# haberdashPI/SignalOperators.jl

Hardware: NVIDIA B200
Metric: sink Msamples/s (Filt+resample+Mix chain) at 1/2/4/8 B200; % of HBM peak (higher is better)
Workload: dtype f64

## Files before the change

### signaloperators.jl_b200/csrc/k_fir_tmap.cuh

```cuda
#pragma once
#include <cuda.h>

#include <type_traits>

#include "k_fir_mma.cuh"

namespace sigops {

constexpr int kFtRows = 128;
constexpr int kFtSlotPos = 16;
constexpr int kFtSlotBytes = kFtRows * 128;
constexpr int kFtMaxSlots = 10;
constexpr int kFtNCW = 8, kFtNAW = 4;
constexpr int kFtThreads = 16 * 32;
constexpr int kFtRegsCompute = 176, kFtRegsHelper = 112, kFtRegsMisc = 40;
constexpr int kFtMaxKs = 64;

struct FirTmParams {
    double* scalars;
    int nscalars, sumsq_slot, nch;
    int64_t nrows, n_out;
    int tapsper;
    int ks;
    int nslot;
    int64_t ntiles, tiles_per_seg;
    const double* pfb;
    const double* dpfb;
    const int64_t* xi0;
    const int32_t* poff;
    const double* alpha;
    int tab_doubles;
    double gain;
    const double* bands_g;
    int period_tiles;
    int64_t epoch_tiles;
    int n_epochs;
    long long* dbg;
    int exp;
};

inline size_t fir_tm_smem_bytes(int nslot, int ks, int tab_doubles, bool has_dpfb) {
    return (size_t)nslot * kFtSlotBytes + 2 * 16384 + (size_t)2 * 4 * ks * 8 * sizeof(double) +
           (size_t)tab_doubles * sizeof(double) * (has_dpfb ? 2 : 1) + 1024;
}

__device__ __forceinline__ void tmap_load_2d(unsigned smem_dst, const CUtensorMap* tm, int c0, int c1, uint64_t* bar) {
    asm volatile("cp.async.bulk.tensor.2d.shared::cluster.global.mbarrier::complete_tx::bytes [%0], [%1, {%2, %3}], [%4];" ::"r"(smem_dst),
                 "l"(tm), "r"(c0), "r"(c1), "r"(smem_u32(bar))
                 : "memory");
}
__device__ __forceinline__ void tmap_store_2d(const CUtensorMap* tm, int c0, int c1, unsigned smem_src) {
    asm volatile("cp.async.bulk.tensor.2d.global.shared::cta.bulk_group [%0, {%1, %2}], [%3];" ::"l"(tm), "r"(c0), "r"(c1), "r"(smem_src)
                 : "memory");
}
__device__ __forceinline__ double lds_f64(unsigned a) {
    double v;
    asm volatile("ld.shared.f64 %0, [%1];" : "=d"(v) : "r"(a));
    return v;
}
__device__ __forceinline__ void sts_f64(unsigned a, double v) { asm volatile("st.shared.f64 [%0], %1;" ::"r"(a), "d"(v) : "memory"); }
__device__ __forceinline__ void sts_v2f64(unsigned a, double x, double y) {
    asm volatile("st.shared.v2.f64 [%0], {%1, %2};" ::"r"(a), "d"(x), "d"(y) : "memory");
}

__device__ __forceinline__ void mbar_wait_a(unsigned bar, unsigned parity) {
    asm volatile(
        "{\n"
        ".reg .pred p;\n"
        "LAB_WAIT:\n"
        "mbarrier.try_wait.parity.shared::cta.b64 p, [%0], %1;\n"
        "@p bra LAB_DONE;\n"
        "bra LAB_WAIT;\n"
        "LAB_DONE:\n"
        "}\n" ::"r"(bar), "r"(parity) : "memory");
}
__device__ __forceinline__ void mbar_arrive_a(unsigned bar) {
    asm volatile("mbarrier.arrive.shared::cta.b64 _, [%0];" ::"r"(bar) : "memory");
}

template <bool SSQ, bool DBG = false>
__global__ void __launch_bounds__(kFtThreads, 1)
k_fir_tmap(const __grid_constant__ FirTmParams P, const __grid_constant__ CUtensorMap tm_in,
           const __grid_constant__ CUtensorMap tm_out) {
    extern __shared__ unsigned char ft_smem_raw[];
    __shared__ uint64_t bar_full[kFtMaxSlots], bar_done[4], bar_taps[2], bar_stg_full[2], bar_stg_free[2];
    __shared__ unsigned done_count;

    const unsigned ring = (smem_u32(ft_smem_raw) + 1023u) & ~1023u;
    const unsigned stg = ring + (unsigned)P.nslot * kFtSlotBytes;
    const unsigned bands = stg + 2 * 16384;
    const unsigned tabs = bands + 2u * 4u * (unsigned)P.ks * 64u;

    const int tid = threadIdx.x, warp = tid >> 5, lane = tid & 31;
    const int row0 = (int)blockIdx.y * kFtRows;
    const int64_t t0 = (int64_t)blockIdx.x * P.tiles_per_seg;
    const int64_t t1 = (t0 + P.tiles_per_seg < P.ntiles) ? t0 + P.tiles_per_seg : P.ntiles;
    if (t0 >= t1) return;

    for (int i = tid; i < P.tab_doubles; i += kFtThreads) {
        sts_f64(tabs + 8u * i, __ldg(P.pfb + i) * P.gain);
        if (P.dpfb) sts_f64(tabs + 8u * (P.tab_doubles + i), __ldg(P.dpfb + i) * P.gain);
    }
    if (tid == 0) {
        done_count = 0u;
        for (int i = 0; i < P.nslot; ++i) mbar_init(&bar_full[i], 1);
        for (int i = 0; i < 4; ++i) mbar_init(&bar_done[i], kFtNCW);
        mbar_init(&bar_taps[0], P.bands_g ? 2 : kFtNAW * 32);
        mbar_init(&bar_taps[1], P.bands_g ? 2 : kFtNAW * 32);
        for (int i = 0; i < 2; ++i) {
            mbar_init(&bar_stg_full[i], kFtNCW / 2);
            mbar_init(&bar_stg_free[i], 1);
        }
        asm volatile("fence.mbarrier_init.release.cluster;" ::: "memory");
    }
    fence_async_smem();
    __syncthreads();

    const int64_t pos_base = (__ldg(P.xi0 + t0 * kFmT) - P.tapsper + 1) & ~int64_t(kFtSlotPos - 1);
    const unsigned band_tile = 4u * (unsigned)P.ks * 64u;

    if (warp < kFtNCW) {
        constexpr int F = 8;
        const int gw = warp & 3, rw = warp >> 2;
        asm volatile("setmaxnreg.inc.sync.aligned.u32 %0;" ::"n"(kFtRegsCompute));
        const int kk = lane & 3, rr = lane >> 2;
        const int rmap = ((rr & 1) << 2) | (rr & 2) | (rr >> 2);
        const int rloc = rw * (8 * F) + rmap;
        const int nn = rr ^ ((kk >> 1) << 2);
        unsigned key = (unsigned)rmap << 4;
        unsigned srow = stg + rloc * 128;
        unsigned bcol = (unsigned)((gw * P.ks + kk) * 64 + nn * 8);
        unsigned arow1 = ring + rloc * 128;
        unsigned ring_end = arow1 + (unsigned)P.nslot * kFtSlotBytes;
        unsigned a_taps = smem_u32(&bar_taps[0]), a_free = smem_u32(&bar_stg_free[rw]), a_full = smem_u32(&bar_stg_full[rw]);
        unsigned a_done = smem_u32(&bar_done[0]), a_cnt = smem_u32(&done_count), lead = lane == 0 ? 1u : 0u;
        asm volatile("" : "+r"(key), "+r"(srow), "+r"(bcol), "+r"(arow1), "+r"(ring_end));
        asm volatile("" : "+r"(a_taps), "+r"(a_free), "+r"(a_full), "+r"(a_done), "+r"(a_cnt), "+r"(lead));
        const int nt = (int)(t1 - t0);
        const int64_t* xp = P.xi0 + t0 * kFmT + 8 * gw;
        double ssq[SSQ ? 8 : 1];
#pragma unroll
        for (int i = 0; i < (SSQ ? 8 : 1); ++i) ssq[i] = 0.0;

        int64_t xq_nx, x7_nx;
        auto fetch_idx = [&](int u) {
            xq_nx = __ldg(xp + (int64_t)u * kFmT);
            x7_nx = __ldg(xp + (int64_t)u * kFmT + 7);
        };
        fetch_idx(0);
        long long dbg_acc[5] = {0, 0, 0, 0, 0};

        unsigned cur = arow1, nxt = arow1;
        int jcur = 0;
        unsigned off[4];
        bool w[4];
        unsigned bq = 0;
        int nbt = 0;
        struct Ops { double a[F], b; };
        Ops o0, o1;

        auto load_ops = [&](Ops& o, auto J) {
            const unsigned ap = (w[J.value] ? nxt : cur) + off[J.value];
#pragma unroll
            for (int i = 0; i < F; ++i) o.a[i] = lds_f64(ap + i * 1024);
            o.b = lds_f64(bq);
            bq += 256;
        };
        auto next_slot = [&]() {
            ++jcur;
            cur = nxt;
            nxt += kFtSlotBytes;
            if (nxt == ring_end) nxt = arow1;
        };
        auto setup = [&](int u, Ops& o) {
            const long long cs = DBG ? clock64() : 0;
            const int s = u & 1;
            const int r = (int)(xq_nx - P.tapsper + 1 - pos_base) + kk;
            int n = (int)(x7_nx - xq_nx) + P.tapsper + 3;
            n >>= 2;
            nbt = n < (P.ks >> 2) ? n : (P.ks >> 2);
            if (u + 1 < nt) fetch_idx(u + 1);
            const int j_new = r >> 4;
            int slot = (int)((cur - arow1) / kFtSlotBytes) + (j_new - jcur);
            while (slot >= P.nslot) slot -= P.nslot;
            while (slot < 0) slot += P.nslot;
            jcur = j_new;
            cur = arow1 + (unsigned)slot * kFtSlotBytes;
            nxt = cur + kFtSlotBytes;
            if (nxt == ring_end) nxt = arow1;
            const unsigned sub0 = (unsigned)(r & 15) << 3;
#pragma unroll
            for (int J = 0; J < 4; ++J) {
                const unsigned q = sub0 + 32u * J;
                w[J] = q >= 128u;
                off[J] = (q & 127u) ^ key;
            }
            bq = bands + s * band_tile + bcol;
            const long long c0 = DBG ? clock64() : 0;
            if (!(P.exp & 16)) mbar_wait_a(a_taps + 8u * s, (unsigned)(u >> 1) & 1u);
            if (DBG) dbg_acc[0] += clock64() - c0;
            load_ops(o, std::integral_constant<int, 0>{});
            if (DBG) dbg_acc[1] += clock64() - cs;
        };
        auto mma_block = [&](double (&acc)[F][2], const Ops& o) {
#pragma unroll
            for (int i = 0; i < F; ++i) dmma884(acc[i][0], acc[i][1], o.a[i], o.b);
        };
        auto stage_store = [&](double (&o)[F][2], int u_old) {
            const long long c0 = DBG ? clock64() : 0;
            if (u_old > 0) mbar_wait_a(a_free, (unsigned)(u_old - 1) & 1u);
            if (DBG) dbg_acc[2] += clock64() - c0;
            if (!(P.exp & 1)) {
                const unsigned sp = srow + (gw >> 1) * 16384 + ((unsigned)(((gw & 1) * 4 + kk) << 4) ^ key);
#pragma unroll
                for (int i = 0; i < F; ++i) sts_v2f64(sp + i * 1024, o[i][0], o[i][1]);
            }
            if (SSQ) {
#pragma unroll
                for (int i = 0; i < F; ++i) ssq[i] = fma(o[i][0], o[i][0], fma(o[i][1], o[i][1], ssq[i]));
            }
            if (DBG) dbg_acc[3] += clock64() - c0;
        };
        auto stage_signal = [&]() {
            const long long c0 = DBG ? clock64() : 0;
            fence_async_smem();
            __syncwarp();
            if (lead) mbar_arrive_a(a_full);
            if (DBG) dbg_acc[3] += clock64() - c0;
        };
        auto tile = [&](double (&acc)[F][2], double (&old)[F][2], int u) {
            const bool more = u + 1 < nt;
#pragma unroll
            for (int i = 0; i < F; ++i) acc[i][0] = acc[i][1] = 0.0;
            const int n = nbt;
            using I0 = std::integral_constant<int, 0>;
            using I1 = std::integral_constant<int, 1>;
            using I2 = std::integral_constant<int, 2>;
            using I3 = std::integral_constant<int, 3>;
            int b = 0;
            bool signalled = u == 0;
            while (true) {
                if (b + 1 < n) {
                    load_ops(o1, I1{});
                    mma_block(acc, o0);
                    if (b == 0 && u > 0) stage_store(old, u - 1);
                } else {
                    if (more) setup(u + 1, o1);
                    mma_block(acc, o0);
                    if (b == 0 && u > 0) stage_store(old, u - 1);
                    o0 = o1;
                    break;
                }
                ++b;
                if (b + 1 < n) {
                    load_ops(o0, I2{});
                    mma_block(acc, o1);
                } else {
                    if (more) setup(u + 1, o0);
                    mma_block(acc, o1);
                    break;
                }
                ++b;
                if (b + 1 < n) {
                    load_ops(o1, I3{});
                    mma_block(acc, o0);
                    if (b == 2 && u > 0) { stage_signal(); signalled = true; }
                } else {
                    if (more) setup(u + 1, o1);
                    mma_block(acc, o0);
                    o0 = o1;
                    break;
                }
                ++b;
                if (b + 1 < n) {
                    next_slot();
                    load_ops(o0, I0{});
                    mma_block(acc, o1);
                } else {
                    if (more) setup(u + 1, o0);
                    mma_block(acc, o1);
                    break;
                }
                ++b;
            }
            if (!signalled) stage_signal();
            __syncwarp();
            if (lead) {
                mbar_arrive_a(a_done + 8u * (u & 3));
                asm volatile("red.release.cta.shared::cta.add.u32 [%0], 1;" ::"r"(a_cnt) : "memory");
            }
        };

        double accA[F][2], accB[F][2];
        setup(0, o0);
        const long long cstart = DBG ? clock64() : 0;
        for (int u = 0; u < nt; u += 2) {
            tile(accA, accB, u);
            if (u + 1 < nt) tile(accB, accA, u + 1);
        }
        if (DBG && warp == 0 && lane == 0) {
            long long* d = P.dbg + ((size_t)blockIdx.y * gridDim.x + blockIdx.x) * 8;
            d[0] = dbg_acc[0]; d[1] = dbg_acc[1]; d[2] = dbg_acc[2]; d[3] = clock64() - cstart; d[6] = dbg_acc[3];
        }
        if (nt & 1) stage_store(accA, nt - 1);
        else stage_store(accB, nt - 1);
        stage_signal();
        if (SSQ) {
#pragma unroll
            for (int i = 0; i < F; ++i) {
                double v = ssq[i];
                v += __shfl_xor_sync(0xffffffffu, v, 1);
                v += __shfl_xor_sync(0xffffffffu, v, 2);
                const int64_t row = (int64_t)row0 + rloc + 8 * i;
                if (kk == 0 && row < P.nrows) atomicAdd(P.scalars + (size_t)(row / P.nch) * P.nscalars + P.sumsq_slot, v);
            }
        }
    } else if (warp < kFtNCW + kFtNAW) {
        asm volatile("setmaxnreg.dec.sync.aligned.u32 %0;" ::"n"(kFtRegsHelper));
        const int grp = warp - kFtNCW;
        if (P.bands_g) {
            if (grp == 0 && lane == 0) {
                const unsigned bytes = 4u * (unsigned)P.ks * 64u;
                int64_t jwait = 0;
                int jw_slot = 0;
                unsigned jw_par = 0;
                for (int64_t t = t0; t < t1; ++t) {
                    const int64_t u = t - t0;
                    const int s = (int)(u & 1);
                    const int64_t hi = (__ldg(P.xi0 + t * kFmT + kFmT - 1) + 4 - pos_base + (kFtSlotPos - 1)) >> 4;
                    if (u >= 2) mbar_wait(&bar_done[(u - 2) & 3], (unsigned)((u - 2) >> 2) & 1u);
                    mbar_expect_tx(&bar_taps[s], bytes);
                    int64_t ep = t / P.epoch_tiles;
                    ep = ep < P.n_epochs ? ep : P.n_epochs - 1;
                    const double* src = P.bands_g + (size_t)(ep * P.period_tiles + t % P.period_tiles) * (bytes / 8);
                    asm volatile("cp.async.bulk.shared::cluster.global.mbarrier::complete_tx::bytes [%0], [%1], %2, [%3];" ::"r"(
                                     bands + (unsigned)s * band_tile),
                                 "l"(src), "r"(bytes), "r"(smem_u32(&bar_taps[s]))
                                 : "memory");
                    while (jwait < hi && !(P.exp & 8)) {
                        mbar_wait(&bar_full[jw_slot], jw_par);
                        ++jwait;
                        if (++jw_slot == P.nslot) { jw_slot = 0; jw_par ^= 1u; }
                    }
                    mbar_arrive(&bar_taps[s]);
                }
            }
            return;
        }
        const int kk = lane & 3, rr = lane >> 2;
        const unsigned pf_tab = tabs, dpf_tab = tabs + 8u * P.tab_doubles;
        const bool has_d = P.dpfb != nullptr;
        const int nblk = P.ks >> 3;
// ... 59 lines not shown
                    const int k = 8 * (b0 + i) + rr;
                    if (b0 + i < nblk) sts_v2f64(band + 8u * (unsigned)(k * 8 + ((2 * kk) ^ (((k >> 1) & 1) << 2))), cv0[i], cv1[i]);
                }
            }
            while (jwait < hi && !(P.exp & 8)) {
                mbar_wait(&bar_full[jw_slot], jw_par);
                ++jwait;
                if (++jw_slot == P.nslot) { jw_slot = 0; jw_par ^= 1u; }
            }
            mbar_arrive(&bar_taps[s]);
            if (DBG) hdbg[1] += clock64() - c1;
        }
        if (DBG && grp == 0 && lane == 0) {
            long long* d = P.dbg + ((size_t)blockIdx.y * gridDim.x + blockIdx.x) * 8;
            d[4] = hdbg[0]; d[5] = hdbg[1];
        }
    } else {
      asm volatile("setmaxnreg.dec.sync.aligned.u32 %0;" ::"n"(kFtRegsMisc));
      if (warp == kFtNCW + kFtNAW) {
        if (lane == 0 && !(P.exp & 8)) {
            const int64_t last_need = __ldg(P.xi0 + (t1 - 1) * kFmT + kFmT - 1) + 4;
            const int64_t nslots_total = (last_need - pos_base + (kFtSlotPos - 1)) >> 4;
            auto lo_of = [&](int64_t t) { return (__ldg(P.xi0 + t * kFmT) - P.tapsper + 1 - pos_base) >> 4; };
            int64_t tp = t0;
            int64_t lo_next = t0 + 1 < t1 ? lo_of(t0 + 1) : (int64_t(1) << 62);
            int s = 0;
            for (int64_t j = 0; j < nslots_total; ++j) {
                if (j >= P.nslot) {
                    const int64_t k = j - P.nslot;
                    while (lo_next <= k) {
                        ++tp;
                        lo_next = tp + 1 < t1 ? lo_of(tp + 1) : (int64_t(1) << 62);
                    }
                    const unsigned target = (unsigned)(tp - t0 + 1) * kFtNCW;
                    unsigned seen;
                    while (true) {
                        asm volatile("ld.acquire.cta.shared::cta.u32 %0, [%1];" : "=r"(seen) : "r"(smem_u32(&done_count)) : "memory");
                        if (seen >= target) break;
                        if (P.exp & 32) __nanosleep(64);
                    }
                }
                mbar_expect_tx(&bar_full[s], kFtSlotBytes);
                tmap_load_2d(ring + (unsigned)s * kFtSlotBytes, &tm_in, (int)(pos_base + j * kFtSlotPos), row0, &bar_full[s]);
                if (++s == P.nslot) s = 0;
            }
        }
      } else {
        const int h = warp - (kFtNCW + kFtNAW + 1);
        if (h < 2 && lane == 0) {
            const bool rows_live = (int64_t)row0 + 64 * h < P.nrows;
            for (int64_t t = t0; t < t1; ++t) {
                const int64_t u = t - t0;
                mbar_wait(&bar_stg_full[h], (unsigned)u & 1u);
                const int64_t m0 = t * kFmT;
                if (!(P.exp & 2) && rows_live) {
                    tmap_store_2d(&tm_out, (int)m0, row0 + 64 * h, stg + 8192u * h);
                    if (m0 + 16 < P.n_out) tmap_store_2d(&tm_out, (int)(m0 + 16), row0 + 64 * h, stg + 16384 + 8192u * h);
                }
                bulk_commit();
                bulk_wait_read_all();
                mbar_arrive(&bar_stg_free[h]);
            }
            bulk_wait_all();
        }
      }
    }
}

}
```

### signaloperators.jl_b200/csrc/runtime.cu

```cuda
#include <algorithm>
#include <array>
#include <atomic>
#include <chrono>
#include <cmath>
#include <cstdarg>
#include <cstdio>
#include <cstdlib>
#include <cstring>
#include <functional>
#include <future>
#include <unordered_map>
#include <memory>
#include <mutex>
#include <string>
#include <thread>
#include <vector>

#include <cuda_runtime.h>

#include "../../include/signalops.h"
#include "common.h"
#include "launchers.h"
#include "k_iir_carry.cuh"
#include "k_fir.cuh"
// ... 147 lines not shown
    bool fast32 = false;
    bool tma_prog = false;
    int prog_in_start = 0, prog_in_len = 0;
    bool rowinv = false;
    std::vector<sigops_instr> rv_in, rv_ep;
    bool unitb = false;
    int n_scale = 0;
    double scale[2] = {1.0, 1.0};
};

struct FirDerived {
    std::vector<int64_t> xi0;
    std::vector<double> phi;
    std::vector<int32_t> poff;
    std::vector<double> alpha;
    int dpad = 0, pmax = 0;
    int pmax32 = 0;
    int ring32 = 0;
    int in_buf = -1;
    int64_t in_len = 0;
    bool epi_const = true;
    double epi_scale = 1.0;
    int64_t period = 0;
    int64_t epoch_tiles = 0;
    int64_t n_epochs = 0;
};

struct StageRT {
    sigops_stage st;
    IirDerived iir;
    FirDerived fir;
};

struct PlanDev {
    bool ready = false;
    sigops_instr* instrs = nullptr;
    double* blob = nullptr;
    std::vector<int64_t*> xi0;
    std::vector<double*> phi;
    std::vector<int32_t*> poff;
    std::vector<double*> alpha;
    std::unordered_map<uint64_t, double*> carry;
    std::unordered_map<uint64_t, double*> bands;
};

}

struct sigops_ctx {
    std::vector<Device> devs;
    std::string err;
    std::mutex mu;
    size_t ws_budget = size_t(16) << 30;
    bool profiling = false;
};

struct sigops_plan {
    sigops_ctx* ctx = nullptr;
    sigops_plan_header h{};
    std::vector<sigops_bufdesc> bufs;
    std::vector<sigops_tabledesc> tables;
    std::vector<sigops_instr> instrs;
    std::vector<sigops_piece> pieces;
    std::vector<StageRT> stages;
    std::vector<double> blob;
    std::vector<PlanDev> dev;
    int nbuf() const { return (int)bufs.size(); }
    int max_stack = 0;
    bool has_randn = false;
    uint64_t uid = 0;
};

namespace {


int program_stack_depth(const sigops_plan& p, int start, int len, bool allow_stage, const char* what) {
    if (len < 0 || start < 0 || (size_t)start + len > p.instrs.size())
// ... 466 lines not shown
    d.phi.assign(p.stages.size(), nullptr);
    d.poff.assign(p.stages.size(), nullptr);
    d.alpha.assign(p.stages.size(), nullptr);
    for (size_t i = 0; i < p.stages.size(); ++i) {
        const FirDerived& f = p.stages[i].fir;
        if (p.stages[i].st.kind != SIGOPS_STAGE_FIR) continue;
        CUDA_OK(cudaMalloc(&d.xi0[i], f.xi0.size() * sizeof(int64_t)));
        CUDA_OK(cudaMalloc(&d.phi[i], f.phi.size() * sizeof(double)));
        CUDA_OK(cudaMemcpy(d.xi0[i], f.xi0.data(), f.xi0.size() * sizeof(int64_t), cudaMemcpyHostToDevice));
        CUDA_OK(cudaMemcpy(d.phi[i], f.phi.data(), f.phi.size() * sizeof(double), cudaMemcpyHostToDevice));
        CUDA_OK(cudaMalloc(&d.poff[i], f.poff.size() * sizeof(int32_t)));
        CUDA_OK(cudaMalloc(&d.alpha[i], f.alpha.size() * sizeof(double)));
        CUDA_OK(cudaMemcpy(d.poff[i], f.poff.data(), f.poff.size() * sizeof(int32_t), cudaMemcpyHostToDevice));
        CUDA_OK(cudaMemcpy(d.alpha[i], f.alpha.data(), f.alpha.size() * sizeof(double), cudaMemcpyHostToDevice));
    }
    d.ready = true;
}

void free_plan_dev(sigops_plan& p) {
    for (size_t di = 0; di < p.dev.size(); ++di) {
        PlanDev& d = p.dev[di];
        if (!d.ready) continue;
        cudaSetDevice(p.ctx->devs[di].ordinal);
        cudaFree(d.instrs);
        cudaFree(d.blob);
        for (auto q : d.xi0) cudaFree(q);
        for (auto q : d.phi) cudaFree(q);
        for (auto q : d.poff) cudaFree(q);
        for (auto q : d.alpha) cudaFree(q);
        for (auto& kv : d.carry) cudaFree(kv.second);
        d.carry.clear();
        for (auto& kv : d.bands) cudaFree(kv.second);
        d.bands.clear();
        d.ready = false;
    }
}


struct IirLaunch {
    int blocks_per_row;
    int64_t L, Wc, nchunks;
    bool need_matrix;
    double cost = 0.0;
};

IirLaunch choose_iir_chunking_flat(const StageRT& s, int64_t rows, int sm_count, bool allow_matrix = true) {
    const int64_t N = s.st.n_out;
    const int64_t W64 = round_up(std::max<int64_t>(s.iir.W, 1), kStageCols);
    const int64_t jmax = std::max<int64_t>(1, (N + kStageCols - 1) / kStageCols);
    double best = 1e300;
    int64_t bestL = kStageCols * jmax;
    const int64_t step = std::max<int64_t>(1, jmax / 4096);
    for (int64_t j = 1; j <= jmax; j += step) {
        const int64_t L = j * kStageCols;
        const int64_t cpr = (N + L - 1) / L;
        const bool matrix = cpr > 1 && W64 >= L;
        if (matrix && !allow_matrix && j + step <= jmax) continue;
        const int64_t blocks = (((rows * cpr) + 31) / 32 + kTmaWarps - 1) / kTmaWarps;
        const int64_t waves = (blocks + sm_count - 1) / sm_count;
        double cost;
        if (matrix) cost = (double)waves * (2.0 * (double)L + 1200.0) + 3.0 * (double)cpr + 400.0;
        else cost = (double)waves * ((double)L + (cpr > 1 ? (double)W64 : 0.0) + 600.0);
        if (N % L) cost *= 1.02;
        if (cost < best) { best = cost; bestL = L; }
    }
    IirLaunch r;
// ... 97 lines not shown
        const BufRef& r = refs[i * nbuf + buf];
        if (((uintptr_t)r.ptr & 15) || (r.nch > 1 && (r.ld & 1)) || (f64 && r.dtype != SIGOPS_F64)) return false;
    }
    return true;
}

bool strided_matrix(const BufRef* refs, int64_t ninst, int nbuf, int buf, int elem_bytes, int dtype, char** base, int64_t* stride) {
    const BufRef& r0 = refs[buf];
    *base = (char*)r0.ptr;
    *stride = r0.ld * elem_bytes;
    if ((*stride & 15) || ((uintptr_t)*base & 15) || r0.dtype != dtype) return false;
    for (int64_t i = 0; i < ninst; ++i) {
        const BufRef& rb = refs[i * nbuf + buf];
        if (rb.ld != r0.ld || rb.nch != r0.nch || rb.dtype != dtype || (char*)rb.ptr != *base + (int64_t)i * r0.nch * *stride)
            return false;
    }
    return true;
}

int64_t choose_tiles_per_segment(int64_t ntiles, int64_t groups, int sm_count) {
    int64_t best_tps = ntiles;
    double best_cost = 1e300;
    for (int w = 1; w <= 8; ++w) {
        int64_t nseg = std::max<int64_t>(1, std::min<int64_t>(ntiles, ((int64_t)w * sm_count + groups - 1) / groups));
        const int64_t tps = (ntiles + nseg - 1) / nseg;
        nseg = (ntiles + tps - 1) / tps;
        const int64_t waves = (groups * nseg + sm_count - 1) / sm_count;
        const double cost = (double)waves * (double)(tps + 3);
        if (cost < best_cost) { best_cost = cost; best_tps = tps; }
    }
    return best_tps;
}

const double* period_bands(const Wave& w, int ks) {
    const uint64_t key = ((uint64_t)w.si << 16) | (uint64_t)ks;
    auto it = w.pd.bands.find(key);
    if (it != w.pd.bands.end()) return it->second;
    const sigops_plan& p = w.p;
    const StageRT& s = p.stages[w.si];
    const sigops_stage& g = s.st;
    const int64_t Pp = s.fir.period;
    const double* hp = p.blob.data() + p.tables[g.pfb_table].offset;
    const double* hd = g.dpfb_table >= 0 ? p.blob.data() + p.tables[g.dpfb_table].offset : nullptr;
    const size_t per_epoch = (size_t)(Pp / 8) * ks * 8;
    std::vector<double> tab(per_epoch * (size_t)s.fir.n_epochs, 0.0);
    for (int64_t e = 0; e < s.fir.n_epochs; ++e) {
        const int64_t start = e * s.fir.epoch_tiles * kFmT;
        for (int64_t q = 0; q < Pp; ++q) {
            const int64_t m = start + q, m0 = m & ~int64_t(7);
            const int n = (int)(m - m0), stn = (int)(s.fir.xi0[m] - s.fir.xi0[m0]);
            double* band = tab.data() + per_epoch * (size_t)e + (size_t)((q & ~int64_t(7)) / 8) * ks * 8;
            for (int t = 0; t < g.taps_per_phase && stn + t < ks; ++t) {
                const double pf = hp[s.fir.poff[m] + t] * s.fir.epi_scale;
                const double h = hd ? std::fma(hd[s.fir.poff[m] + t] * s.fir.epi_scale, s.fir.alpha[m], pf) : pf;
                const int k = stn + t;
                band[k * 8 + (n ^ (((k >> 1) & 1) << 2))] = h;
            }
        }
    }
    double* dptr = nullptr;
    CUDA_OK(cudaMalloc(&dptr, tab.size() * sizeof(double)));
    CUDA_OK(cudaMemcpy(dptr, tab.data(), tab.size() * sizeof(double), cudaMemcpyHostToDevice));
    w.pd.bands.emplace(key, dptr);
    return dptr;
}

std::array<double, 8> fir_cycles_per_tile(cudaStream_t stream, size_t nblocks, int64_t tiles_per_seg,
                                          const std::function<void(long long*)>& launch) {
    long long* dbg = nullptr;
    CUDA_OK(cudaMalloc(&dbg, nblocks * 8 * sizeof(long long)));
    CUDA_OK(cudaMemset(dbg, 0, nblocks * 8 * sizeof(long long)));
    launch(dbg);
    CUDA_OK(cudaStreamSynchronize(stream));
    std::vector<long long> h(nblocks * 8);
    CUDA_OK(cudaMemcpy(h.data(), dbg, h.size() * sizeof(long long), cudaMemcpyDeviceToHost));
    cudaFree(dbg);
    std::array<double, 8> sum{};
    for (size_t b = 0; b < nblocks; ++b)
        for (int k = 0; k < 8; ++k) sum[k] += (double)h[b * 8 + k];
    const double per = 1.0 / ((double)nblocks * (double)tiles_per_seg);
    for (double& v : sum) v *= per;
    return sum;
}

template <class... P, class... A>
void launch_dyn_smem(void (*kernel)(P...), dim3 grid, int threads, size_t smem, cudaStream_t st, const A&... args) {
    ensure_dyn_smem(kernel, smem);
    kernel<<<grid, threads, smem, st>>>(args...);
}

void plan_map_stage(const Wave& w) {
    const sigops_plan& p = w.p;
    const sigops_stage& g = p.stages[w.si].st;
    MapParams P{};
    P.instrs = w.pd.instrs; P.bufrefs = w.d_refs; P.scalars = w.scalars; P.inst0 = w.inst0;
    P.nbuf = w.nbuf; P.nscalars = w.nscal;
    P.out_buf = g.out_buf; P.sumsq_slot = g.sumsq_slot; P.out_nch = p.bufs[g.out_buf].nchannels;
// ... 144 lines not shown
    if (c.nchunks <= 1 || warm) return;
    if (c.need_matrix) {
        CarryParams C{};
        C.state_zs = P.state_zs; C.state_in = P.state_in;
        C.nrows = rows; C.slots_per_row = P.slots_per_row; C.nchunks = c.nchunks; C.M2 = S;
        const uint64_t akey = ((uint64_t)w.si << 40) ^ (uint64_t)c.L;
        double*& dAL = w.pd.carry[akey];
        if (!dAL) {
            std::vector<double> AL = transition_matrix(P.coef, s.iir.M, c.L);
            CUDA_OK(cudaMalloc(&dAL, AL.size() * sizeof(double)));
            CUDA_OK(cudaMemcpy(dAL, AL.data(), AL.size() * sizeof(double), cudaMemcpyHostToDevice));
        }
        C.AL = dAL;
        const unsigned cblocks = (unsigned)((rows + 3) / 4);
        w.add(KIND_IIR_CARRY, [=](cudaStream_t st) { k_iir_carry<<<cblocks, 128, 0, st>>>(C); });
    }
    w.add(KIND_IIR_FIX, [=](cudaStream_t st) {
        if (tma) launch_iir_tma_any(LAUNCH_FIX, false, M_, unitb, grid, st, Q);
        else if (fast) launch_iir_cpasync(LAUNCH_FIX, M_, unitb, grid, st, P);
        else launch_iir_generic(LAUNCH_FIX, M_, grid, stack_iir, st, P);
    });
}

bool plan_fir_tmap(const Wave& w, const FirParams& P) {
    const StageRT& s = w.p.stages[w.si];
    const sigops_stage& g = s.st;
    const int64_t rows = P.nrows;
    if (rows <= 64 || getenv("SIGOPS_NO_FIR_TMAP") || !iir_tmap_available() || rows >= (int64_t(1) << 31) ||
        g.n_out >= (int64_t(1) << 31) || s.fir.in_len >= (int64_t(1) << 31))
        return false;
    const int ks = (int)round_up(s.fir.dpad + g.taps_per_phase, 8);
    const int win_slots = (s.fir.pmax32 + 3 + 14) / 16 + 1;
    const bool has_d = P.dpfb != nullptr;
    const double* bands_g = nullptr;
    int period_tiles = 0;
    if (s.fir.period > 0 && g.sumsq_slot < 0 && !getenv("SIGOPS_NO_FIR_BANDS") &&
        (size_t)(s.fir.period / 8) * ks * 64 * (size_t)s.fir.n_epochs <= (size_t(96) << 20)) {
        bands_g = period_bands(w, ks);
        period_tiles = (int)(s.fir.period / kFmT);
    }
    const int64_t tabd = bands_g ? 0 : (int64_t)g.n_phases * g.taps_per_phase;
    int nslot = kFtMaxSlots;
    while (nslot > win_slots + 1 && fir_tm_smem_bytes(nslot, ks, (int)tabd, has_d) > kFirTmSmemLimit) --nslot;
    char *bin = nullptr, *bout = nullptr;
    int64_t sin_ = 0, sout = 0;
    TensorMapBlob mi, mo;
    if (!(ks <= kFtMaxKs && nslot >= win_slots + 1 && fir_tm_smem_bytes(nslot, ks, (int)tabd, has_d) <= kFirTmSmemLimit &&
          strided_matrix(w.refs, w.ninst, w.nbuf, s.fir.in_buf, 8, SIGOPS_F64, &bin, &sin_) &&
          strided_matrix(w.refs, w.ninst, w.nbuf, g.out_buf, 8, SIGOPS_F64, &bout, &sout) && s.fir.in_len >= 1 &&
          tmap_encode_2d_f64(&mi, bin, s.fir.in_len, rows, sin_, kFtSlotPos, kFtRows) &&
          tmap_encode_2d_f64(&mo, bout, g.n_out, rows, sout, 16, kFtRows / 2)))
        return false;
    FirTmParams T{};
    T.scalars = w.scalars; T.nscalars = w.nscal; T.sumsq_slot = g.sumsq_slot; T.nch = g.nchannels;
    T.nrows = rows; T.n_out = g.n_out; T.tapsper = g.taps_per_phase; T.ks = ks; T.nslot = nslot;
    T.ntiles = (g.n_out + kFmT - 1) / kFmT;
    T.pfb = P.pfb; T.dpfb = P.dpfb; T.xi0 = P.xi0; T.poff = w.pd.poff[w.si]; T.alpha = w.pd.alpha[w.si];
    T.tab_doubles = (int)tabd;
    T.bands_g = bands_g; T.period_tiles = period_tiles;
    T.epoch_tiles = s.fir.epoch_tiles; T.n_epochs = (int)s.fir.n_epochs;
    T.gain = s.fir.epi_scale;
    if (const char* e = getenv("SIGOPS_FIR_EXP")) T.exp = atoi(e);
    const int64_t groups = (rows + kFtRows - 1) / kFtRows;
    if (groups > 65535) return false;
    T.tiles_per_seg = choose_tiles_per_segment(T.ntiles, groups, w.sm_count);
    const int64_t nseg = (T.ntiles + T.tiles_per_seg - 1) / T.tiles_per_seg;
    const size_t smem = fir_tm_smem_bytes(nslot, ks, (int)tabd, has_d);
    dim3 tgrid((unsigned)nseg, (unsigned)groups);
    if (getenv("SIGOPS_DEBUG")) {
        fprintf(stderr, "[sigops] FIR stage %zu: tensor-map rows=%lld n_out=%lld taps=%d ks=%d slots=%d (window %d) grid=%lldx%lld tiles/seg=%lld smem=%zu gain=%g period=%lld outputs%s\n",
                w.si, (long long)rows, (long long)g.n_out, T.tapsper, ks, nslot, win_slots, (long long)nseg, (long long)groups,
                (long long)T.tiles_per_seg, smem, T.gain, (long long)s.fir.period, bands_g ? " (tap bands from the period tables)" : "");
        if (bands_g) fprintf(stderr, "[sigops]   %lld epochs of %lld tiles\n", (long long)s.fir.n_epochs, (long long)s.fir.epoch_tiles);
    }
    if (getenv("SIGOPS_FIR_DBG")) {
        const auto c = fir_cycles_per_tile(w.stream, (size_t)nseg * groups, T.tiles_per_seg, [&](long long* dbg) {
            FirTmParams D = T;
            D.dbg = dbg;
            launch_dyn_smem(k_fir_tmap<false, true>, tgrid, kFtThreads, smem, w.stream, D, *(const CUtensorMap*)&mi,
                            *(const CUtensorMap*)&mo);
        });
        fprintf(stderr, "[sigops] FIR tmap cycles/tile  compute: set-up %.0f (of it wait_taps %.0f) staging %.0f (of it wait_stg %.0f) total %.0f | helper: wait_done %.0f build %.0f\n",
                c[1], c[0], c[6], c[2], c[3], c[4], c[5]);
    }
    const auto kernel = g.sumsq_slot >= 0 ? k_fir_tmap<true> : k_fir_tmap<false>;
    w.add(KIND_FIR, [=](cudaStream_t st) {
        launch_dyn_smem(kernel, tgrid, kFtThreads, smem, st, T, *(const CUtensorMap*)&mi, *(const CUtensorMap*)&mo);
    });
    return true;
}

bool plan_fir_mma(const Wave& w, const FirParams& P) {
    const StageRT& s = w.p.stages[w.si];
    const sigops_stage& g = s.st;
    const int64_t rows = P.nrows;
    FirMmaParams Q{};
    Q.bufrefs = w.d_refs; Q.scalars = w.scalars; Q.nbuf = w.nbuf; Q.nscalars = w.nscal;
    Q.in_buf = s.fir.in_buf; Q.out_buf = g.out_buf; Q.sumsq_slot = g.sumsq_slot;
    Q.in_len = s.fir.in_len; Q.nch = g.nchannels; Q.nrows = rows; Q.n_out = g.n_out;
    Q.tapsper = g.taps_per_phase;
    Q.ks = (int)round_up(s.fir.dpad + g.taps_per_phase, 4);
    Q.ring = s.fir.ring32;
    Q.pitch = Q.ring + ((4 - Q.ring % 16) + 16) % 16;
    Q.pfb = P.pfb; Q.dpfb = P.dpfb; Q.xi0 = P.xi0; Q.poff = w.pd.poff[w.si]; Q.alpha = w.pd.alpha[w.si];
    Q.ntiles = (g.n_out + kFmT - 1) / kFmT;
    Q.gain = s.fir.epi_scale;
    const int64_t tabd = (int64_t)g.n_phases * g.taps_per_phase;
    const size_t tab_bytes = (size_t)tabd * 8 * (P.dpfb ? 2 : 1);
    Q.tab_doubles = (int)tabd;
    if (tab_bytes > 48 * 1024) return false;
    auto smem_for = [&](int RBx) {
        return (size_t)RBx * Q.pitch * 8 + (size_t)2 * 4 * Q.ks * kFmHbPitch * 8 + tab_bytes;
    };
    int RB = rows > 64 ? 128 : (rows > 32 ? 64 : 32);
    while (RB > 32 && smem_for(RB) > kFirMmaSmemLimit) RB >>= 1;
    const int64_t groups = (rows + RB - 1) / RB;
    if (smem_for(RB) > kFirMmaSmemLimit || groups > 65535) return false;
    Q.tiles_per_seg = choose_tiles_per_segment(Q.ntiles, groups, w.sm_count);
// ... 874 lines not shown
```

Baseline: 276,900.

## Keep periodic FIR tap bands resident in Blackwell tensor memory

For periodic resampling stages, the precomputed tap bands for the current and next epoch are loaded once per block into tensor memory (tcgen05 alloc/st). The compute warps then read the B operand with tcgen05.ld instead of shared memory, and leading all-zero tap rows are trimmed per group. This removes the helper warps that streamed bands into shared memory and their per-tile barrier handshake, and frees shared memory for a deeper input ring (12 slots). Other changes: per-warp done counters replace a single shared counter, and segments are capped to one epoch. The costs are added complexity, tensor-memory alloc/dealloc, a bounded period size, and host-side band trimming with validation.

```diff
diff --git a/signaloperators.jl_b200/csrc/k_fir_tmap.cuh b/signaloperators.jl_b200/csrc/k_fir_tmap.cuh
--- a/signaloperators.jl_b200/csrc/k_fir_tmap.cuh
+++ b/signaloperators.jl_b200/csrc/k_fir_tmap.cuh
@@ -10,7 +10,9 @@
 constexpr int kFtRows = 128;
 constexpr int kFtSlotPos = 16;
 constexpr int kFtSlotBytes = kFtRows * 128;
-constexpr int kFtMaxSlots = 10;
+constexpr int kFtMaxSlots = 12;
+constexpr int kFtMaxSlotsSmemBands = 10;
+constexpr int kFtTmMaxPT = 32;
 constexpr int kFtNCW = 8, kFtNAW = 4;
 constexpr int kFtThreads = 16 * 32;
 constexpr int kFtRegsCompute = 176, kFtRegsHelper = 112, kFtRegsMisc = 40;
@@ -35,11 +37,16 @@
     int period_tiles;
     int64_t epoch_tiles;
     int n_epochs;
+    const double* tm_img;
+    const uint8_t* tm_lead;
+    int tm_nblk;
+    int tm_cols;
     long long* dbg;
     int exp;
 };
 
-inline size_t fir_tm_smem_bytes(int nslot, int ks, int tab_doubles, bool has_dpfb) {
+inline size_t fir_tm_smem_bytes(int nslot, int ks, int tab_doubles, bool has_dpfb, bool tmem = false) {
+    if (tmem) return (size_t)nslot * kFtSlotBytes + 2 * 16384 + 1024;
     return (size_t)nslot * kFtSlotBytes + 2 * 16384 + (size_t)2 * 4 * ks * 8 * sizeof(double) +
            (size_t)tab_doubles * sizeof(double) * (has_dpfb ? 2 : 1) + 1024;
 }
@@ -61,6 +68,17 @@
 __device__ __forceinline__ void sts_f64(unsigned a, double v) { asm volatile("st.shared.f64 [%0], %1;" ::"r"(a), "d"(v) : "memory"); }
 __device__ __forceinline__ void sts_v2f64(unsigned a, double x, double y) {
     asm volatile("st.shared.v2.f64 [%0], {%1, %2};" ::"r"(a), "d"(x), "d"(y) : "memory");
+}
+
+__device__ __forceinline__ void tmem_st_f64(unsigned taddr, double v) {
+    asm volatile("tcgen05.st.sync.aligned.32x32b.x2.b32 [%0], {%1, %2};" ::"r"(taddr), "r"(__double2loint(v)), "r"(__double2hiint(v))
+                 : "memory");
+}
+__device__ __forceinline__ void tmem_ld_f64(unsigned taddr, unsigned& lo, unsigned& hi) {
+    asm volatile("tcgen05.ld.sync.aligned.32x32b.x2.b32 {%0, %1}, [%2];" : "=r"(lo), "=r"(hi) : "r"(taddr));
+}
+__device__ __forceinline__ void tmem_wait_ld(unsigned& lo, unsigned& hi) {
+    asm volatile("tcgen05.wait::ld.sync.aligned;" : "+r"(lo), "+r"(hi)::"memory");
 }
 
 __device__ __forceinline__ void mbar_wait_a(unsigned bar, unsigned parity) {
@@ -78,13 +96,15 @@
     asm volatile("mbarrier.arrive.shared::cta.b64 _, [%0];" ::"r"(bar) : "memory");
 }
 
-template <bool SSQ, bool DBG = false>
+template <bool SSQ, bool DBG = false, bool TM = false>
 __global__ void __launch_bounds__(kFtThreads, 1)
 k_fir_tmap(const __grid_constant__ FirTmParams P, const __grid_constant__ CUtensorMap tm_in,
            const __grid_constant__ CUtensorMap tm_out) {
     extern __shared__ unsigned char ft_smem_raw[];
     __shared__ uint64_t bar_full[kFtMaxSlots], bar_done[4], bar_taps[2], bar_stg_full[2], bar_stg_free[2];
-    __shared__ unsigned done_count;
+    __shared__ unsigned done_w[kFtNCW];
+    __shared__ unsigned tm_base_sh;
+    __shared__ uint8_t tm_lead_sh[2 * kFtTmMaxPT * 4];
 
     const unsigned ring = (smem_u32(ft_smem_raw) + 1023u) & ~1023u;
     const unsigned stg = ring + (unsigned)P.nslot * kFtSlotBytes;
@@ -101,8 +121,14 @@
         sts_f64(tabs + 8u * i, __ldg(P.pfb + i) * P.gain);
         if (P.dpfb) sts_f64(tabs + 8u * (P.tab_doubles + i), __ldg(P.dpfb + i) * P.gain);
     }
+    if (TM && warp == kFtNCW) {
+        asm volatile("tcgen05.alloc.cta_group::1.sync.aligned.shared::cta.b32 [%0], %1;" ::"r"(smem_u32(&tm_base_sh)), "r"(P.tm_cols)
+                     : "memory");
+        asm volatile("tcgen05.relinquish_alloc_permit.cta_group::1.sync.aligned;" ::: "memory");
+        asm volatile("tcgen05.fence::before_thread_sync;" ::: "memory");
+    }
     if (tid == 0) {
-        done_count = 0u;
+        for (int i = 0; i < kFtNCW; ++i) done_w[i] = 0u;
         for (int i = 0; i < P.nslot; ++i) mbar_init(&bar_full[i], 1);
         for (int i = 0; i < 4; ++i) mbar_init(&bar_done[i], kFtNCW);
         mbar_init(&bar_taps[0], P.bands_g ? 2 : kFtNAW * 32);
@@ -115,6 +141,7 @@
     }
     fence_async_smem();
     __syncthreads();
+    if (TM) asm volatile("tcgen05.fence::after_thread_sync;" ::: "memory");
 
     const int64_t pos_base = (__ldg(P.xi0 + t0 * kFmT) - P.tapsper + 1) & ~int64_t(kFtSlotPos - 1);
     const unsigned band_tile = 4u * (unsigned)P.ks * 64u;
@@ -133,10 +160,38 @@
         unsigned arow1 = ring + rloc * 128;
         unsigned ring_end = arow1 + (unsigned)P.nslot * kFtSlotBytes;
         unsigned a_taps = smem_u32(&bar_taps[0]), a_free = smem_u32(&bar_stg_free[rw]), a_full = smem_u32(&bar_stg_full[rw]);
-        unsigned a_done = smem_u32(&bar_done[0]), a_cnt = smem_u32(&done_count), lead = lane == 0 ? 1u : 0u;
+        unsigned a_done = smem_u32(&bar_done[0]), a_cnt = smem_u32(&done_w[warp]), lead = lane == 0 ? 1u : 0u;
         asm volatile("" : "+r"(key), "+r"(srow), "+r"(bcol), "+r"(arow1), "+r"(ring_end));
         asm volatile("" : "+r"(a_taps), "+r"(a_free), "+r"(a_full), "+r"(a_done), "+r"(a_cnt), "+r"(lead));
         const int nt = (int)(t1 - t0);
+
+        const int nb2 = 2 * P.tm_nblk;
+        int tpc = 0;
+        int u_ep = 1 << 30;
+        unsigned tq = 0, ecol = 0, elead = 0;
+        int jw = 0;
+        unsigned jw_bar = smem_u32(&bar_full[0]), jw_par = 0;
+        if (TM) {
+            const int PT = P.period_tiles;
+            const int ep0 = (int)min(t0 / P.epoch_tiles, (int64_t)P.n_epochs - 1);
+            const int ne = ep0 + 1 < P.n_epochs ? 2 : 1;
+            if (ne == 2) u_ep = (int)((int64_t)(ep0 + 1) * P.epoch_tiles - t0);
+            tpc = (int)(t0 % PT);
+            tq = tm_base_sh + ((unsigned)(32 * gw) << 16);
+            if (rw == 0) {
+                const double* src = P.tm_img + ((size_t)ep0 * PT * 4 + gw) * P.tm_nblk * 32 + lane;
+                for (int i = 0; i < ne * PT; ++i) {
+                    const double* sp = src + (size_t)i * 4 * P.tm_nblk * 32;
+#pragma unroll 4
+                    for (int b = 0; b < P.tm_nblk; ++b) tmem_st_f64(tq + (unsigned)(i * nb2 + 2 * b), __ldg(sp + 32 * b));
+                }
+                for (int i = lane; i < ne * PT; i += 32) tm_lead_sh[i * 4 + gw] = __ldg(P.tm_lead + ((size_t)ep0 * PT + i) * 4 + gw);
+                asm volatile("tcgen05.wait::st.sync.aligned;" ::: "memory");
+            }
+            asm volatile("tcgen05.fence::before_thread_sync;" ::: "memory");
+            asm volatile("bar.sync 1, %0;" ::"n"(kFtNCW * 32) : "memory");
+            asm volatile("tcgen05.fence::after_thread_sync;" ::: "memory");
+        }
         const int64_t* xp = P.xi0 + t0 * kFmT + 8 * gw;
         double ssq[SSQ ? 8 : 1];
 #pragma unroll
@@ -156,15 +211,24 @@
         bool w[4];
         unsigned bq = 0;
         int nbt = 0;
-        struct Ops { double a[F], b; };
+        struct Ops { double a[F], b; unsigned blo, bhi; };
         Ops o0, o1;
 
         auto load_ops = [&](Ops& o, auto J) {
             const unsigned ap = (w[J.value] ? nxt : cur) + off[J.value];
+            if (TM) {
+                tmem_ld_f64(bq, o.blo, o.bhi);
+                bq += 2;
+            }
 #pragma unroll
             for (int i = 0; i < F; ++i) o.a[i] = lds_f64(ap + i * 1024);
-            o.b = lds_f64(bq);
-            bq += 256;
+            if (!TM) {
+                o.b = lds_f64(bq);
+                bq += 256;
+            }
+        };
+        auto b_ready = [&](Ops& o) {
+            if (TM) tmem_wait_ld(o.blo, o.bhi);
         };
         auto next_slot = [&]() {
             ++jcur;
@@ -175,10 +239,22 @@
         auto setup = [&](int u, Ops& o) {
             const long long cs = DBG ? clock64() : 0;
             const int s = u & 1;
-            const int r = (int)(xq_nx - P.tapsper + 1 - pos_base) + kk;
-            int n = (int)(x7_nx - xq_nx) + P.tapsper + 3;
+            int lz = 0;
+            if (TM) {
+                if (u == u_ep) {
+                    ecol = (unsigned)(P.period_tiles * nb2);
+                    elead = (unsigned)(P.period_tiles * 4);
+                }
+                lz = tm_lead_sh[elead + tpc * 4 + gw];
+                bq = tq + ecol + (unsigned)(tpc * nb2);
+                if (++tpc == P.period_tiles) tpc = 0;
+            }
+            const int r = (int)(xq_nx - P.tapsper + 1 - pos_base) + kk + lz;
+            int n = (int)(x7_nx - xq_nx) + P.tapsper - lz + 3;
             n >>= 2;
-            nbt = n < (P.ks >> 2) ? n : (P.ks >> 2);
+            const int nmax = TM ? P.tm_nblk : (P.ks >> 2);
+            nbt = n < nmax ? n : nmax;
+            const int hi = TM ? (int)((x7_nx + 4 - pos_base + (kFtSlotPos - 1)) >> 4) : 0;
             if (u + 1 < nt) fetch_idx(u + 1);
             const int j_new = r >> 4;
             int slot = (int)((cur - arow1) / kFtSlotBytes) + (j_new - jcur);
@@ -195,16 +271,29 @@
                 w[J] = q >= 128u;
                 off[J] = (q & 127u) ^ key;
             }
-            bq = bands + s * band_tile + bcol;
             const long long c0 = DBG ? clock64() : 0;
-            if (!(P.exp & 16)) mbar_wait_a(a_taps + 8u * s, (unsigned)(u >> 1) & 1u);
+            if (TM) {
+#pragma unroll 1
+                while (jw < hi && !(P.exp & 8)) {
+                    mbar_wait_a(jw_bar, jw_par);
+                    ++jw;
+                    jw_bar += 8u;
+                    if (jw_bar == smem_u32(&bar_full[0]) + 8u * (unsigned)P.nslot) {
+                        jw_bar = smem_u32(&bar_full[0]);
+                        jw_par ^= 1u;
+                    }
+                }
+            } else {
+                bq = bands + s * band_tile + bcol;
+                if (!(P.exp & 16)) mbar_wait_a(a_taps + 8u * s, (unsigned)(u >> 1) & 1u);
+            }
             if (DBG) dbg_acc[0] += clock64() - c0;
             load_ops(o, std::integral_constant<int, 0>{});
             if (DBG) dbg_acc[1] += clock64() - cs;
         };
         auto mma_block = [&](double (&acc)[F][2], const Ops& o) {
 #pragma unroll
-            for (int i = 0; i < F; ++i) dmma884(acc[i][0], acc[i][1], o.a[i], o.b);
+            for (int i = 0; i < F; ++i) dmma884(acc[i][0], acc[i][1], o.a[i], TM ? __hiloint2double(o.bhi, o.blo) : o.b);
         };
         auto stage_store = [&](double (&o)[F][2], int u_old) {
             const long long c0 = DBG ? clock64() : 0;
@@ -244,10 +333,12 @@
                     load_ops(o1, I1{});
                     mma_block(acc, o0);
                     if (b == 0 && u > 0) stage_store(old, u - 1);
+                    b_ready(o1);
                 } else {
                     if (more) setup(u + 1, o1);
                     mma_block(acc, o0);
                     if (b == 0 && u > 0) stage_store(old, u - 1);
+                    b_ready(o1);
                     o0 = o1;
                     break;
                 }
@@ -255,9 +346,11 @@
                 if (b + 1 < n) {
                     load_ops(o0, I2{});
                     mma_block(acc, o1);
+                    b_ready(o0);
                 } else {
                     if (more) setup(u + 1, o0);
                     mma_block(acc, o1);
+                    b_ready(o0);
                     break;
                 }
                 ++b;
@@ -265,9 +358,11 @@
                     load_ops(o1, I3{});
                     mma_block(acc, o0);
                     if (b == 2 && u > 0) { stage_signal(); signalled = true; }
+                    b_ready(o1);
                 } else {
                     if (more) setup(u + 1, o1);
                     mma_block(acc, o0);
+                    b_ready(o1);
                     o0 = o1;
                     break;
                 }
@@ -276,9 +371,11 @@
                     next_slot();
                     load_ops(o0, I0{});
                     mma_block(acc, o1);
+                    b_ready(o0);
                 } else {
                     if (more) setup(u + 1, o0);
                     mma_block(acc, o1);
+                    b_ready(o0);
                     break;
                 }
                 ++b;
@@ -286,13 +383,14 @@
             if (!signalled) stage_signal();
             __syncwarp();
             if (lead) {
-                mbar_arrive_a(a_done + 8u * (u & 3));
+                if (!TM) mbar_arrive_a(a_done + 8u * (u & 3));
                 asm volatile("red.release.cta.shared::cta.add.u32 [%0], 1;" ::"r"(a_cnt) : "memory");
             }
         };
 
         double accA[F][2], accB[F][2];
         setup(0, o0);
+        b_ready(o0);
         const long long cstart = DBG ? clock64() : 0;
         for (int u = 0; u < nt; u += 2) {
             tile(accA, accB, u);
@@ -315,9 +413,21 @@
                 if (kk == 0 && row < P.nrows) atomicAdd(P.scalars + (size_t)(row / P.nch) * P.nscalars + P.sumsq_slot, v);
             }
         }
+        if (TM) {
+            asm volatile("tcgen05.fence::before_thread_sync;" ::: "memory");
+            asm volatile("bar.arrive 2, %0;" ::"n"((kFtNCW + 1) * 32) : "memory");
+        }
     } else if (warp < kFtNCW + kFtNAW) {
         asm volatile("setmaxnreg.dec.sync.aligned.u32 %0;" ::"n"(kFtRegsHelper));
         const int grp = warp - kFtNCW;
+        if (TM) {
+            if (grp == 0) {
+                asm volatile("bar.sync 2, %0;" ::"n"((kFtNCW + 1) * 32) : "memory");
+                asm volatile("tcgen05.fence::after_thread_sync;" ::: "memory");
+                asm volatile("tcgen05.dealloc.cta_group::1.sync.aligned.b32 %0, %1;" ::"r"(tm_base_sh), "r"(P.tm_cols) : "memory");
+            }
+            return;
+        }
         if (P.bands_g) {
             if (grp == 0 && lane == 0) {
                 const unsigned bytes = 4u * (unsigned)P.ks * 64u;
@@ -443,12 +553,14 @@
                         ++tp;
                         lo_next = tp + 1 < t1 ? lo_of(tp + 1) : (int64_t(1) << 62);
                     }
-                    const unsigned target = (unsigned)(tp - t0 + 1) * kFtNCW;
-                    unsigned seen;
-                    while (true) {
-                        asm volatile("ld.acquire.cta.shared::cta.u32 %0, [%1];" : "=r"(seen) : "r"(smem_u32(&done_count)) : "memory");
-                        if (seen >= target) break;
-                        if (P.exp & 32) __nanosleep(64);
+                    const unsigned target = (unsigned)(tp - t0 + 1);
+                    for (int cw = 0; cw < kFtNCW; ++cw) {
+                        unsigned seen;
+                        while (true) {
+                            asm volatile("ld.acquire.cta.shared::cta.u32 %0, [%1];" : "=r"(seen) : "r"(smem_u32(&done_w[cw])) : "memory");
+                            if (seen >= target) break;
+                            if (P.exp & 32) __nanosleep(64);
+                        }
                     }
                 }
                 mbar_expect_tx(&bar_full[s], kFtSlotBytes);
diff --git a/signaloperators.jl_b200/csrc/runtime.cu b/signaloperators.jl_b200/csrc/runtime.cu
--- a/signaloperators.jl_b200/csrc/runtime.cu
+++ b/signaloperators.jl_b200/csrc/runtime.cu
@@ -203,6 +203,12 @@
     FirDerived fir;
 };
 
+struct TmBands {
+    double* img = nullptr;
+    const uint8_t* lead = nullptr;
+    int nblk = 0;
+};
+
 struct PlanDev {
     bool ready = false;
     sigops_instr* instrs = nullptr;
@@ -213,6 +219,7 @@
     std::vector<double*> alpha;
     std::unordered_map<uint64_t, double*> carry;
     std::unordered_map<uint64_t, double*> bands;
+    std::unordered_map<uint64_t, TmBands> tm_bands;
 };
 
 }
@@ -745,6 +752,8 @@
         d.carry.clear();
         for (auto& kv : d.bands) cudaFree(kv.second);
         d.bands.clear();
+        for (auto& kv : d.tm_bands) cudaFree(kv.second.img);
+        d.tm_bands.clear();
         d.ready = false;
     }
 }
@@ -908,30 +917,38 @@
     return best_tps;
 }
 
+void merged_band(const Wave& w, int64_t m0, int ks, double* band) {
+    const sigops_plan& p = w.p;
+    const StageRT& s = p.stages[w.si];
+    const sigops_stage& g = s.st;
+    const double* hp = p.blob.data() + p.tables[g.pfb_table].offset;
+    const double* hd = g.dpfb_table >= 0 ? p.blob.data() + p.tables[g.dpfb_table].offset : nullptr;
+    std::fill(band, band + (size_t)ks * 8, 0.0);
+    for (int n = 0; n < 8; ++n) {
+        const int64_t m = m0 + n;
+        const int stn = (int)(s.fir.xi0[m] - s.fir.xi0[m0]);
+        for (int t = 0; t < g.taps_per_phase && stn + t < ks; ++t) {
+            const double pf = hp[s.fir.poff[m] + t] * s.fir.epi_scale;
+            band[(stn + t) * 8 + n] = hd ? std::fma(hd[s.fir.poff[m] + t] * s.fir.epi_scale, s.fir.alpha[m], pf) : pf;
+        }
+    }
+}
+
 const double* period_bands(const Wave& w, int ks) {
     const uint64_t key = ((uint64_t)w.si << 16) | (uint64_t)ks;
     auto it = w.pd.bands.find(key);
     if (it != w.pd.bands.end()) return it->second;
-    const sigops_plan& p = w.p;
-    const StageRT& s = p.stages[w.si];
-    const sigops_stage& g = s.st;
+    const StageRT& s = w.p.stages[w.si];
     const int64_t Pp = s.fir.period;
-    const double* hp = p.blob.data() + p.tables[g.pfb_table].offset;
-    const double* hd = g.dpfb_table >= 0 ? p.blob.data() + p.tables[g.dpfb_table].offset : nullptr;
     const size_t per_epoch = (size_t)(Pp / 8) * ks * 8;
-    std::vector<double> tab(per_epoch * (size_t)s.fir.n_epochs, 0.0);
+    std::vector<double> tab(per_epoch * (size_t)s.fir.n_epochs, 0.0), band((size_t)ks * 8);
     for (int64_t e = 0; e < s.fir.n_epochs; ++e) {
         const int64_t start = e * s.fir.epoch_tiles * kFmT;
-        for (int64_t q = 0; q < Pp; ++q) {
-            const int64_t m = start + q, m0 = m & ~int64_t(7);
-            const int n = (int)(m - m0), stn = (int)(s.fir.xi0[m] - s.fir.xi0[m0]);
-            double* band = tab.data() + per_epoch * (size_t)e + (size_t)((q & ~int64_t(7)) / 8) * ks * 8;
-            for (int t = 0; t < g.taps_per_phase && stn + t < ks; ++t) {
-                const double pf = hp[s.fir.poff[m] + t] * s.fir.epi_scale;
-                const double h = hd ? std::fma(hd[s.fir.poff[m] + t] * s.fir.epi_scale, s.fir.alpha[m], pf) : pf;
-                const int k = stn + t;
-                band[k * 8 + (n ^ (((k >> 1) & 1) << 2))] = h;
-            }
+        for (int64_t q = 0; q < Pp; q += 8) {
+            merged_band(w, start + q, ks, band.data());
+            double* dst = tab.data() + per_epoch * (size_t)e + (size_t)(q / 8) * ks * 8;
+            for (int k = 0; k < ks; ++k)
+                for (int n = 0; n < 8; ++n) dst[k * 8 + (n ^ (((k >> 1) & 1) << 2))] = band[k * 8 + n];
         }
     }
     double* dptr = nullptr;
@@ -939,6 +956,55 @@
     CUDA_OK(cudaMemcpy(dptr, tab.data(), tab.size() * sizeof(double), cudaMemcpyHostToDevice));
     w.pd.bands.emplace(key, dptr);
     return dptr;
+}
+
+TmBands period_bands_tm(const Wave& w, int ks) {
+    const uint64_t key = ((uint64_t)w.si << 16) | (uint64_t)ks;
+    auto it = w.pd.tm_bands.find(key);
+    if (it != w.pd.tm_bands.end()) return it->second;
+    const StageRT& s = w.p.stages[w.si];
+    const int tapsper = s.st.taps_per_phase;
+    const int64_t Pp = s.fir.period, ngrp = s.fir.n_epochs * (Pp / 8);
+    std::vector<double> bands((size_t)ngrp * ks * 8);
+    std::vector<uint8_t> lead((size_t)ngrp);
+    int nblk = 0;
+    for (int64_t e = 0; e < s.fir.n_epochs; ++e)
+        for (int64_t q = 0; q < Pp; q += 8) {
+            const int64_t i = e * (Pp / 8) + q / 8, m0 = e * s.fir.epoch_tiles * kFmT + q;
+            double* band = bands.data() + (size_t)i * ks * 8;
+            merged_band(w, m0, ks, band);
+            const int span = (int)(s.fir.xi0[m0 + 7] - s.fir.xi0[m0]) + tapsper;
+            auto row_zero = [&](int k) {
+                for (int n = 0; n < 8; ++n)
+                    if (band[k * 8 + n] != 0.0) return false;
+                return true;
+            };
+            int l = 0;
+            while (l < ks && row_zero(l)) ++l;
+            const int nsteps = (span - l + 3) / 4;
+            for (int k = l + 4 * nsteps; k < ks; ++k)
+                if (!row_zero(k))
+                    fail(SIGOPS_ERR_INVALID, "internal: trimmed tap band of tile %lld, group %lld drops row %d",
+                         (long long)(m0 / kFmT), (long long)((m0 / 8) & 3), k);
+            lead[(size_t)i] = (uint8_t)l;
+            nblk = std::max(nblk, nsteps);
+        }
+    std::vector<double> img((size_t)ngrp * nblk * 32, 0.0);
+    for (int64_t i = 0; i < ngrp; ++i)
+        for (int b = 0; b < nblk; ++b)
+            for (int ln = 0; ln < 32; ++ln) {
+                const int k = lead[(size_t)i] + 4 * b + (ln & 3);
+                if (k < ks) img[((size_t)i * nblk + b) * 32 + ln] = bands[((size_t)i * ks + k) * 8 + (ln >> 2)];
+            }
+    TmBands t;
+    t.nblk = nblk;
+    const size_t img_bytes = img.size() * sizeof(double);
+    CUDA_OK(cudaMalloc(&t.img, img_bytes + lead.size()));
+    CUDA_OK(cudaMemcpy(t.img, img.data(), img_bytes, cudaMemcpyHostToDevice));
+    CUDA_OK(cudaMemcpy((char*)t.img + img_bytes, lead.data(), lead.size(), cudaMemcpyHostToDevice));
+    t.lead = (const uint8_t*)((char*)t.img + img_bytes);
+    w.pd.tm_bands.emplace(key, t);
+    return t;
 }
 
 std::array<double, 8> fir_cycles_per_tile(cudaStream_t stream, size_t nblocks, int64_t tiles_per_seg,
@@ -1149,20 +1215,29 @@
     const int ks = (int)round_up(s.fir.dpad + g.taps_per_phase, 8);
     const int win_slots = (s.fir.pmax32 + 3 + 14) / 16 + 1;
     const bool has_d = P.dpfb != nullptr;
+    const bool periodic = s.fir.period > 0 && g.sumsq_slot < 0 && !getenv("SIGOPS_NO_FIR_BANDS") &&
+                          (size_t)(s.fir.period / 8) * ks * 64 * (size_t)s.fir.n_epochs <= (size_t(96) << 20);
+    const int period_tiles = periodic ? (int)(s.fir.period / kFmT) : 0;
+    const int64_t eps = s.fir.n_epochs > 1 ? 2 : 1;
+    const bool tm = periodic && !getenv("SIGOPS_NO_FIR_TMEM") && period_tiles <= kFtTmMaxPT &&
+                    period_tiles * 2 * (ks / 4) * eps <= 256;
     const double* bands_g = nullptr;
-    int period_tiles = 0;
-    if (s.fir.period > 0 && g.sumsq_slot < 0 && !getenv("SIGOPS_NO_FIR_BANDS") &&
-        (size_t)(s.fir.period / 8) * ks * 64 * (size_t)s.fir.n_epochs <= (size_t(96) << 20)) {
+    TmBands tmb;
+    int tm_cols = 0;
+    if (tm) {
+        tmb = period_bands_tm(w, ks);
+        tm_cols = 32;
+        while (tm_cols < period_tiles * 2 * tmb.nblk * eps) tm_cols *= 2;
+    } else if (periodic) {
         bands_g = period_bands(w, ks);
-        period_tiles = (int)(s.fir.period / kFmT);
-    }
-    const int64_t tabd = bands_g ? 0 : (int64_t)g.n_phases * g.taps_per_phase;
-    int nslot = kFtMaxSlots;
-    while (nslot > win_slots + 1 && fir_tm_smem_bytes(nslot, ks, (int)tabd, has_d) > kFirTmSmemLimit) --nslot;
+    }
+    const int64_t tabd = periodic ? 0 : (int64_t)g.n_phases * g.taps_per_phase;
+    int nslot = tm ? kFtMaxSlots : kFtMaxSlotsSmemBands;
+    while (nslot > win_slots + 1 && fir_tm_smem_bytes(nslot, ks, (int)tabd, has_d, tm) > kFirTmSmemLimit) --nslot;
     char *bin = nullptr, *bout = nullptr;
     int64_t sin_ = 0, sout = 0;
     TensorMapBlob mi, mo;
-    if (!(ks <= kFtMaxKs && nslot >= win_slots + 1 && fir_tm_smem_bytes(nslot, ks, (int)tabd, has_d) <= kFirTmSmemLimit &&
+    if (!(ks <= kFtMaxKs && nslot >= win_slots + 1 && fir_tm_smem_bytes(nslot, ks, (int)tabd, has_d, tm) <= kFirTmSmemLimit &&
           strided_matrix(w.refs, w.ninst, w.nbuf, s.fir.in_buf, 8, SIGOPS_F64, &bin, &sin_) &&
           strided_matrix(w.refs, w.ninst, w.nbuf, g.out_buf, 8, SIGOPS_F64, &bout, &sout) && s.fir.in_len >= 1 &&
           tmap_encode_2d_f64(&mi, bin, s.fir.in_len, rows, sin_, kFtSlotPos, kFtRows) &&
@@ -1176,31 +1251,35 @@
     T.tab_doubles = (int)tabd;
     T.bands_g = bands_g; T.period_tiles = period_tiles;
     T.epoch_tiles = s.fir.epoch_tiles; T.n_epochs = (int)s.fir.n_epochs;
+    T.tm_img = tmb.img; T.tm_lead = tmb.lead; T.tm_nblk = tmb.nblk; T.tm_cols = tm_cols;
     T.gain = s.fir.epi_scale;
     if (const char* e = getenv("SIGOPS_FIR_EXP")) T.exp = atoi(e);
     const int64_t groups = (rows + kFtRows - 1) / kFtRows;
     if (groups > 65535) return false;
     T.tiles_per_seg = choose_tiles_per_segment(T.ntiles, groups, w.sm_count);
+    if (tm) T.tiles_per_seg = std::min(T.tiles_per_seg, s.fir.epoch_tiles);
     const int64_t nseg = (T.ntiles + T.tiles_per_seg - 1) / T.tiles_per_seg;
-    const size_t smem = fir_tm_smem_bytes(nslot, ks, (int)tabd, has_d);
+    const size_t smem = fir_tm_smem_bytes(nslot, ks, (int)tabd, has_d, tm);
     dim3 tgrid((unsigned)nseg, (unsigned)groups);
     if (getenv("SIGOPS_DEBUG")) {
-        fprintf(stderr, "[sigops] FIR stage %zu: tensor-map rows=%lld n_out=%lld taps=%d ks=%d slots=%d (window %d) grid=%lldx%lld tiles/seg=%lld smem=%zu gain=%g period=%lld outputs%s\n",
+        char tmdesc[96] = "";
+        if (tm) snprintf(tmdesc, sizeof tmdesc, " (tap bands in tensor memory: %d columns, %d k-blocks, staging x1)", tm_cols, tmb.nblk);
+        fprintf(stderr, "[sigops] FIR stage %zu: tensor-map rows=%lld n_out=%lld taps=%d ks=%d slots=%d (window %d) grid=%lldx%lld tiles/seg=%lld smem=%zu gain=%g%s period=%lld outputs%s\n",
                 w.si, (long long)rows, (long long)g.n_out, T.tapsper, ks, nslot, win_slots, (long long)nseg, (long long)groups,
-                (long long)T.tiles_per_seg, smem, T.gain, (long long)s.fir.period, bands_g ? " (tap bands from the period tables)" : "");
-        if (bands_g) fprintf(stderr, "[sigops]   %lld epochs of %lld tiles\n", (long long)s.fir.n_epochs, (long long)s.fir.epoch_tiles);
+                (long long)T.tiles_per_seg, smem, T.gain, tmdesc, (long long)s.fir.period, periodic ? " (tap bands from the period tables)" : "");
+        if (periodic) fprintf(stderr, "[sigops]   %lld epochs of %lld tiles\n", (long long)s.fir.n_epochs, (long long)s.fir.epoch_tiles);
     }
     if (getenv("SIGOPS_FIR_DBG")) {
         const auto c = fir_cycles_per_tile(w.stream, (size_t)nseg * groups, T.tiles_per_seg, [&](long long* dbg) {
             FirTmParams D = T;
             D.dbg = dbg;
-            launch_dyn_smem(k_fir_tmap<false, true>, tgrid, kFtThreads, smem, w.stream, D, *(const CUtensorMap*)&mi,
-                            *(const CUtensorMap*)&mo);
+            launch_dyn_smem(tm ? k_fir_tmap<false, true, true> : k_fir_tmap<false, true>, tgrid, kFtThreads, smem, w.stream, D,
+                            *(const CUtensorMap*)&mi, *(const CUtensorMap*)&mo);
         });
         fprintf(stderr, "[sigops] FIR tmap cycles/tile  compute: set-up %.0f (of it wait_taps %.0f) staging %.0f (of it wait_stg %.0f) total %.0f | helper: wait_done %.0f build %.0f\n",
                 c[1], c[0], c[6], c[2], c[3], c[4], c[5]);
     }
-    const auto kernel = g.sumsq_slot >= 0 ? k_fir_tmap<true> : k_fir_tmap<false>;
+    const auto kernel = tm ? k_fir_tmap<false, false, true> : g.sumsq_slot >= 0 ? k_fir_tmap<true> : k_fir_tmap<false>;
     w.add(KIND_FIR, [=](cudaStream_t st) {
         launch_dyn_smem(kernel, tgrid, kFtThreads, smem, st, T, *(const CUtensorMap*)&mi, *(const CUtensorMap*)&mo);
     });
```

Result: faster. 282,300, median of 6 (+1.9%).
